# Lakonik/MVEdit

Hardware: AMD Instinct MI355X
Metric: multi-view denoise-steps/sec (32 views, 512^2) (higher is better)
Workload: dtype f16; 1 GPU; 32-view 512x512 get_noise_pred: 64 SD-1.5 UNet forwards (64x64 latents, ctx 77x768) + CFG per step; ControlNet residuals zero; views=32, latent=64, cfg=True, parallelism=views/1

## Files before the change

### include/mvedit_amd.h

```cpp
#ifndef MVEDIT_AMD_H
#define MVEDIT_AMD_H

#include <stdint.h>
#include <stddef.h>

#ifdef __cplusplus
extern "C" {
#endif

#define MVE_API __attribute__((visibility("default")))

typedef enum {
    MVE_OK = 0,
    MVE_ERR_ARG = -1,
    MVE_ERR_HIP = -2,
    MVE_ERR_STATE = -3,
    MVE_ERR_NOMEM = -4
} mve_status;

typedef enum {
    MVE_F32 = 0,
    MVE_F16 = 1,
    MVE_BF16 = 2,
    MVE_I32 = 3,
// ... 5 lines not shown
MVE_API int mve_device_info(int* n_cu, int* wave_size, char* arch, int arch_len);


MVE_API int mve_near_far_from_aabb(const float* d_rays_o, const float* d_rays_d, const float* d_aabb,
                                   uint32_t N, float min_near, float* d_nears, float* d_fars, void* stream);

MVE_API int mve_morton3d(const int32_t* d_coords, uint32_t N, int32_t* d_indices, void* stream);
MVE_API int mve_morton3d_invert(const int32_t* d_indices, uint32_t N, int32_t* d_coords, void* stream);

MVE_API int mve_packbits(const float* d_grid, uint32_t n_bytes, float density_thresh, uint8_t* d_bitfield, void* stream);

MVE_API int mve_flatten_rays(const int32_t* d_rays, uint32_t N, uint32_t M, int32_t* d_res, void* stream);

MVE_API size_t mve_march_scratch_bytes(uint32_t N);
MVE_API int mve_march_rays_train_count(const float* d_rays_o, const float* d_rays_d, const uint8_t* d_grid,
                                       float bound, int contract, float dt_gamma, uint32_t max_steps,
                                       uint32_t N, uint32_t C, uint32_t H,
                                       const float* d_nears, const float* d_fars, const float* d_noises,
                                       int32_t* d_rays, int32_t* d_total, void* d_scratch, void* stream);
MVE_API int mve_march_rays_train_write(const float* d_rays_o, const float* d_rays_d, const uint8_t* d_grid,
                                       float bound, int contract, float dt_gamma, uint32_t max_steps,
                                       uint32_t N, uint32_t C, uint32_t H,
                                       const float* d_nears, const float* d_fars, const float* d_noises,
                                       const int32_t* d_rays, uint32_t capacity,
                                       float* d_xyzs, float* d_dirs, float* d_ts, void* stream);

MVE_API int mve_march_rays_train_clamp(const int32_t* d_rays, uint32_t N, const int32_t* d_total, uint32_t capacity,
                                       int32_t* d_n_samples, int32_t* d_count, int32_t* d_overflow, void* stream);

MVE_API int mve_composite_rays_train_forward(const float* d_sigmas, const float* d_rgbs, const float* d_ts,
                                             const int32_t* d_rays, uint32_t M, uint32_t N, float T_thresh, int binarize,
                                             float* d_weights, float* d_weights_sum, float* d_depth, float* d_image,
                                             void* stream);
MVE_API int mve_composite_rays_train_backward(const float* d_grad_weights, const float* d_grad_weights_sum,
                                              const float* d_grad_depth, const float* d_grad_image,
                                              const float* d_sigmas, const float* d_rgbs, const float* d_ts,
                                              const int32_t* d_rays, const float* d_weights_sum, const float* d_depth,
                                              const float* d_image, uint32_t M, uint32_t N, float T_thresh, int binarize,
                                              float* d_grad_sigmas, float* d_grad_rgbs, void* stream);

MVE_API int mve_march_rays(uint32_t n_alive, uint32_t n_step, const int32_t* d_rays_alive, const float* d_rays_t,
                           const float* d_rays_o, const float* d_rays_d, float bound, int contract, float dt_gamma,
                           uint32_t max_steps, uint32_t C, uint32_t H, const uint8_t* d_grid,
                           const float* d_nears, const float* d_fars,
                           float* d_xyzs, float* d_dirs, float* d_ts, const float* d_noises, void* stream);
MVE_API int mve_composite_rays(uint32_t n_alive, uint32_t n_step, float T_thresh, int binarize,
                               int32_t* d_rays_alive, float* d_rays_t, const float* d_sigmas, const float* d_rgbs,
                               const float* d_ts, float* d_weights_sum, float* d_depth, float* d_image, void* stream);

MVE_API int mve_compact_alive(const int32_t* d_rays_alive, uint32_t n_alive, int32_t* d_out, int32_t* d_n_out,
                              void* d_scratch, void* stream);

MVE_API size_t mve_cull_scratch_bytes(uint32_t M);
MVE_API int mve_cull_samples(const float* d_weights, uint32_t M, float threshold, const int32_t* d_rays, uint32_t N,
                             const float* d_xyzs, const float* d_dirs, const float* d_ts, float* d_out_xyzs, float* d_out_dirs,
                             float* d_out_ts, int32_t* d_out_rays, int32_t* d_pref, int32_t* d_n_out, void* d_scratch,
                             void* stream);
MVE_API int mve_cull_samples_n(const float* d_weights, uint32_t capacity, const int32_t* d_count, float threshold, const int32_t* d_rays,
                               uint32_t N, const float* d_xyzs, const float* d_dirs, const float* d_ts, float* d_out_xyzs,
                               float* d_out_dirs, float* d_out_ts, int32_t* d_out_rays, int32_t* d_pref, int32_t* d_n_out,
                               void* d_scratch, void* stream);

MVE_API int mve_density_grid_points(const int32_t* d_coords, const float* d_noise, uint32_t N, uint32_t grid_size, float bound,
                                    float* d_xyzs, int32_t* d_indices, void* stream);
MVE_API size_t mve_density_grid_scratch_bytes(uint32_t n_cells);
MVE_API int mve_density_grid_update(float* d_density_grid, float* d_tmp_grid, uint32_t n_cells, const float* d_sigmas,
                                    const int32_t* d_indices, uint32_t N, float decay, float* d_mean_density, void* d_scratch,
                                    void* stream);


#define MVE_GEMM_GEGLU   1
#define MVE_GEMM_OUT_F32 2
#define MVE_CONV_W_CHUNK64 4
#define MVE_GEMM_NO_SPLITK 8
#define MVE_CONV_PAD_BR 32
#define MVE_GEMM_RES_AFTER_SCALE 16

MVE_API int mve_gemm(int dtype, const void* d_A, int lda, const void* d_W, int ldw, void* d_out, int ldc,
                     int M, int N, int K, const float* d_bias, const float* d_rowvec, int ldrv, int rows_per_vec,
                     const void* d_residual, int ldr, int flags, float out_scale, void* d_workspace,
                     size_t workspace_bytes, int rows_per_image, void* stream);

MVE_API int mve_gemm_tune(int big_min_blocks);
MVE_API int mve_gemm_red_tune(int on);
MVE_API int mve_gemm_deep_tune(int max_blocks);
MVE_API int mve_gemm_effective_splitk(int M, int N, int K, int rows_per_image);
#define MVE_PLAN_RESIDUAL 1
#define MVE_PLAN_RESIDUAL_LO 2
#define MVE_PLAN_OUT_LO 4
#define MVE_PLAN_ROWVEC 8
#define MVE_PLAN_LN 16
#define MVE_PLAN_BIAS 32
#define MVE_PLAN_WORKSPACE 64
#define MVE_PLAN_SCALED 128
#define MVE_PLAN_DESCRIBE_INTS 12
MVE_API int mve_gemm_plan_describe(int kind, int M, int N, int K, int rows_per_image, int flags, int features, const int* conv_geom, int* out);

MVE_API int mve_gemm_pp_profile(void* d_buf);

MVE_API size_t mve_gemm_workspace_bytes(int M, int N, int K, int rows_per_image);

MVE_API int mve_conv3x3(int dtype, const void* d_x1, int C1, const void* d_x2, int C2, int B, int Hs, int Ws,
                        int stride, int upsample, const void* d_W, int Cout, void* d_out, int ldc,
                        const float* d_bias, const float* d_rowvec, int ldrv, const void* d_residual, int ldr,
                        int flags, float out_scale, void* d_workspace, size_t workspace_bytes, void* stream);

MVE_API int mve_conv3x3_shortcut(int dtype, const void* x1, int C1, const void* x3, int C3, const void* x4, int C4, int B, int Hs,
                                 int Ws, const void* W, int Cout, void* out, int ldc, const float* bias, const float* bias2,
                                 const void* residual, int ldr, int flags, float out_scale, void* d_workspace,
                                 size_t workspace_bytes, void* stream);

MVE_API int mve_upsample_conv_phases_supported(int C, int Cout, int B, int Hs, int Ws);
MVE_API int mve_upsample_conv_phases_tune(int one_launch);
MVE_API size_t mve_upsample_conv_phases_workspace_bytes(int C, int Cout, int B, int Hs, int Ws);
MVE_API int mve_pack_upsample_phase_weights(int src_dtype, int dst_dtype, const void* d_w_oihw, int Cout, int C, void* d_W4, void* stream);
MVE_API int mve_upsample_conv_phases(int dtype, const void* d_x, int C, int B, int Hs, int Ws, const void* d_W4, int Cout, void* d_out,
                                     const float* d_bias, int flags, void* d_workspace, size_t workspace_bytes, void* d_out_lo, void* stream);

MVE_API int mve_gemm_pair(int dtype, const void* d_A, int lda, const void* d_W, int ldw, void* d_out, int ldc,
                          int M, int N, int K, const float* d_bias, const float* d_rowvec, int ldrv, int rows_per_vec,
                          const void* d_residual, int ldr, int flags, float out_scale, void* d_workspace,
                          size_t workspace_bytes, int rows_per_image, const void* d_residual_lo, void* d_out_lo, void* stream);

MVE_API int mve_gemm_pair_ln(int dtype, const void* d_A, int lda, const void* d_W, int ldw, void* d_out, int ldc, int M, int N, int K,
                             const float* d_bias, const void* d_residual, int ldr, void* d_workspace, size_t workspace_bytes, int rows_per_image,
                             const void* d_residual_lo, void* d_out_lo, void* d_ln_out, int ld_ln, const float* d_ln_gamma, const float* d_ln_beta,
                             float ln_eps, void* stream);
MVE_API int mve_gemm_ln_fuse_tune(int on);

MVE_API int mve_conv3x3_pair(int dtype, const void* x1, int C1, const void* x2, int C2, int B, int Hs, int Ws, int stride,
                             int upsample, const void* W, int Cout, void* out, int ldc, const float* bias, const float* rowvec,
                             int ldrv, const void* residual, int ldr, int flags, float out_scale, void* d_workspace,
                             size_t workspace_bytes, const void* d_residual_lo, void* d_out_lo, void* stream);
MVE_API int mve_conv3x3_shortcut_pair(int dtype, const void* x1, int C1, const void* x3, int C3, const void* x4, int C4, int B, int Hs,
                                      int Ws, const void* W, int Cout, void* out, int ldc, const float* bias, const float* bias2,
                                      int flags, float out_scale, void* d_workspace, size_t workspace_bytes, void* d_out_lo, void* stream);
MVE_API int mve_groupnorm_silu_pair(int dtype, const void* d_x1, int C1, const void* d_x2, int C2, int B, int HW, int G,
                                    float eps, const float* d_gamma, const float* d_beta, int silu, void* d_out,
                                    void* d_workspace, const void* d_x1_lo, const void* d_x2_lo, void* stream);
MVE_API int mve_layernorm_pair(int dtype, const void* d_x, int ldx, void* d_y, int ldy, int M, int C,
                               const float* d_gamma, const float* d_beta, float eps, const void* d_x_lo, void* stream);
MVE_API int mve_axpy_pair(int dtype, const void* d_a, const void* d_a_lo, const void* d_b, float alpha, void* d_y, void* d_y_lo, size_t n, void* stream);

MVE_API int mve_mxfp8_packed_k(int K);
MVE_API int mve_mxfp8_quantize(int dtype, const void* d_x, int ldx, int R, int K, uint8_t* d_q, uint8_t* d_e, void* stream);
MVE_API int mve_mxfp8_gemm(const uint8_t* d_aq, const uint8_t* d_ae, const uint8_t* d_wq, const uint8_t* d_we, int M, int N, int K, int out_dtype,
                           void* d_out, int ldc, const float* d_bias, const void* d_residual, int ldr, void* stream);

MVE_API int mve_attention(int dtype, const void* d_Q, int ldq, const void* d_K, int ldk, const void* d_V, int ldv,
                          const void* d_K2, int ldk2, const void* d_V2, int ldv2, void* d_O, int ldo,
                          int B, int Lq, int Lk, int Lk2, int heads, int head_dim, float scale, void* stream);
MVE_API int mve_attention_tune(int variant);
MVE_API int mve_attention_profile(unsigned long long* out4);
MVE_API int mve_attention_prescaled(int dtype, const void* d_Q, int ldq, const void* d_K, int ldk, const void* d_V, int ldv,
                                    const void* d_K2, int ldk2, const void* d_V2, int ldv2, void* d_O, int ldo,
                                    int B, int Lq, int Lk, int Lk2, int heads, int head_dim, void* stream);


MVE_API int mve_attention_causal(int dtype, const void* d_Q, int ldq, const void* d_K, int ldk, const void* d_V, int ldv, void* d_O, int ldo,
                                 int B, int L, int heads, int head_dim, float scale, void* stream);
MVE_API int mve_clip_embed(int dtype, const int32_t* d_ids, const void* d_tok, const void* d_pos, void* d_out, int B, int L, int C, int vocab,
                           int max_pos, void* stream);
#define MVE_ACT_QUICK_GELU 0
#define MVE_ACT_GELU 1
MVE_API int mve_act(int dtype, int kind, const void* d_x, void* d_y, size_t n, void* stream);
MVE_API int mve_clip_pool(int dtype, const void* d_x, const int32_t* d_ids, void* d_out, int B, int L, int C, int eos_token_id, void* stream);


MVE_API int mve_clip_patchify(int dtype, const void* d_pixels, int B, int H, int W, int P, void* d_rows, int ld, void* stream);
MVE_API int mve_clip_vision_embed(int dtype, const void* d_patch, const void* d_cls, const void* d_pos, void* d_out, int B, int G2, int C, void* stream);


MVE_API int mve_dpt_stem_rows(int dtype, const void* d_pixels, int B, int S, void* d_rows, int ld, void* stream);
MVE_API int mve_dpt_maxpool(int dtype, const void* d_x, int B, int H, int W, int C, void* d_y, void* stream);
MVE_API int mve_dpt_gather_s2(int dtype, const void* d_x, int B, int H, int W, int C, void* d_y, void* stream);
MVE_API int mve_dpt_upsample2x(int dtype, const void* d_x, int B, int H, int W, int C, void* d_y, void* stream);
MVE_API int mve_dpt_add_relu(int dtype, const void* d_a, const void* d_b, void* d_y, size_t n, void* stream);


MVE_API int mve_loftr_stem_rows(int dtype, const void* d_pixels, int B, int H, int W, void* d_rows, int ld, void* stream);
MVE_API int mve_loftr_leaky_relu(int dtype, const void* d_x, void* d_y, size_t n, float slope, void* stream);
MVE_API int mve_loftr_pos_add(int dtype, const void* d_x, const float* d_pos, void* d_y, int B, int HW, int C, void* stream);

MVE_API size_t mve_linattn_workspace_bytes(int B, int S, int H, int D);
MVE_API int mve_linattn_kv(int dtype, const void* d_k, int ldk, const void* d_v, int ldv, int B, int S, int H, int D, float* d_kv, void* d_workspace,
                           size_t workspace_bytes, void* stream);
MVE_API int mve_linattn_apply(int dtype, const void* d_q, int ldq, const float* d_kv, void* d_out, int ldo, int B, int L, int H, int D, float eps,
                              void* stream);

MVE_API int mve_dsmax_stats(const float* d_sim, int N, int L, int S, int ld, float* d_row_stats, float* d_col_stats, void* stream);
MVE_API int mve_dsmax_conf(const float* d_sim, int N, int L, int S, int ld, const float* d_row_stats, const float* d_col_stats, float* d_conf, void* stream);
MVE_API size_t mve_dsmax_select_workspace_bytes(int N, int L, int S);
MVE_API int mve_dsmax_select(const float* d_conf, int N, int H0, int W0, int H1, int W1, float thr, int border, float scale, int64_t* d_b_ids,
                             int64_t* d_i_ids, int64_t* d_j_ids, float* d_mconf, float* d_mkpts0_c, float* d_mkpts1_c, int* d_count, void* d_workspace,
                             size_t workspace_bytes, void* stream);

MVE_API int mve_loftr_unfold(int dtype, const void* d_feat, int N, int Hf, int Wf, int C, const int64_t* d_b_ids, const int64_t* d_ids, int M, void* d_rows,
                             void* stream);
MVE_API int mve_loftr_ln_add(int dtype, const void* d_o, int ldo, const void* d_x, int ldx, void* d_y, int ldy, int M, int C, const float* d_gamma,
                             const float* d_beta, float eps, void* stream);
MVE_API int mve_loftr_gather_rows(int dtype, const void* d_feat, int N, int L, int C, const int64_t* d_b_ids, const int64_t* d_ids, int M, void* d_rows,
                                  void* stream);
MVE_API int mve_loftr_fine_match(int dtype, const void* d_feat0, const void* d_feat1, int M, int C, const float* d_mkpts1_c, float radius, float* d_expec_f,
                                 float* d_mkpts1_f, void* stream);


MVE_API int mve_attention_relpos(int dtype, const void* d_Q, int ldq, const void* d_K, int ldk, const void* d_V, int ldv, const void* d_rel_h,
                                 const void* d_rel_w, void* d_O, int ldo, int NS, int gh, int gw, int heads, int head_dim, float scale, void* stream);
MVE_API int mve_sam_window_partition(int dtype, const void* d_x, int B, int G, int C, int window, void* d_win, void* stream);
MVE_API int mve_sam_window_unpartition(int dtype, const void* d_win, int B, int G, int C, int window, void* d_x, void* stream);
MVE_API int mve_sam_pos_add(int dtype, const void* d_x, const void* d_pos, void* d_y, int B, int HW, int C, void* stream);


MVE_API int mve_sam_preprocess(int dtype, const uint8_t* d_image, int h, int w, int S, const float* pixel_mean, const float* pixel_std, void* d_out, void* stream);
MVE_API int mve_sam_dense_pe(const float* d_gaussian, float* d_out, int G, int C, void* stream);
MVE_API int mve_sam_prompt_tokens(const float* d_boxes, const float* d_points, const int32_t* d_labels, int N, int n_points, const float* d_gaussian,
                                  const float* d_point_embed, const float* d_not_a_point, const float* d_iou_token, const float* d_mask_tokens, int num_mask_tokens,
                                  int C, float image_size, float* d_out, int T, void* stream);
MVE_API int mve_sam_src(int dtype, const void* d_embedding, const float* d_no_mask_embed, float* d_out, int N, int P, int C, int G, void* stream);
MVE_API int mve_gemm_f32(const float* d_A, int lda, const float* d_W, int ldw, const float* d_bias, const float* d_res, int ldr, float* d_out, int ldc, int M, int N,
                         int K, int relu, void* stream);
MVE_API int mve_attention_f32(const float* d_Q, int ldq, const float* d_K, int ldk, const float* d_V, int ldv, float* d_O, int ldo, int NB, int Lq, int Lk,
                              int heads, int head_dim, float scale, void* stream);
MVE_API int mve_layernorm_f32(const float* d_x, float* d_y, int rows, int C, const float* d_gamma, const float* d_beta, float eps, void* stream);
MVE_API int mve_add_rows_f32(const float* d_x, const float* d_pe, float* d_y, int rows, int C, int period_rows, void* stream);
MVE_API int mve_sam_upscale(const float* d_x, const float* d_W4, const float* d_bias, const float* d_ln_gamma, const float* d_ln_beta, float eps, float* d_tmp,
                            float* d_out, int N, int Gi, int Cin, int Cout, int mode, void* stream);
MVE_API int mve_sam_token_mlps(const float* d_queries, int N, int T, int C, int hidden, int out_dim, int num_mask_tokens, const float* d_w0, const float* d_b0,
                               const float* d_w1, const float* d_b1, const float* d_w2, const float* d_b2, float* d_hyper, float* d_iou, void* stream);
MVE_API int mve_sam_mask_product(const float* d_hyper, const float* d_up, float* d_low_res, int N, int num_mask_tokens, int Cu, int pixels, void* stream);
MVE_API int mve_sam_postprocess(const float* d_low_res, int planes, int L, int S, int h_in, int w_in, int H, int W, float mask_threshold, uint8_t* d_masks,
                                float* d_logits, void* stream);

MVE_API int mve_groupnorm_tune(int fused_max_hw);
MVE_API size_t mve_groupnorm_workspace_bytes(int B, int HW, int C, int G);
MVE_API int mve_groupnorm_silu(int dtype, const void* d_x1, int C1, const void* d_x2, int C2, int B, int HW, int G,
                               float eps, const float* d_gamma, const float* d_beta, int silu, void* d_out,
                               void* d_workspace, void* stream);

MVE_API int mve_layernorm(int dtype, const void* d_x, int ldx, void* d_y, int ldy, int M, int C,
                          const float* d_gamma, const float* d_beta, float eps, void* stream);

MVE_API int mve_nchw_to_nhwc(int dst_dtype, int src_dtype, const void* d_x, int B, int C, int H, int W, int Cpad,
                             void* d_y, void* stream);
MVE_API int mve_nhwc_to_nchw(int dst_dtype, int src_dtype, const void* d_x, int ld, int B, int C, int H, int W,
                             void* d_y, void* stream);
MVE_API int mve_timestep_embedding(int dtype, const float* d_t, int B, int dim, void* d_out, void* stream);
MVE_API int mve_text_time_embedding(int dtype, const void* d_text_embeds, int text_dtype, int text_dim, const float* d_time_ids, int n_ids,
                                    int time_embed_dim, int B, void* d_out, void* stream);
MVE_API int mve_silu(int dtype, const void* d_x, void* d_y, size_t n, void* stream);
MVE_API int mve_axpy(int dtype, const void* d_a, const void* d_b, float alpha, void* d_y, size_t n, void* stream);
MVE_API int mve_softmax_rows(int dtype, const float* d_scores, size_t lds, int M, int N, void* d_probs, size_t ldp, void* stream);
MVE_API int mve_cfg_combine(const float* d_uncond, const float* d_text, float guidance_scale, float* d_out, size_t n,
                            void* stream);
MVE_API int mve_x0_prediction(const float* d_latents_scaled, const float* d_noise_pred, float sqrt_alpha_bar,
                              float sqrt_one_minus_alpha_bar, size_t n, float* d_x0, void* stream);

MVE_API int mve_tonemap_lut(const float* d_x, size_t n, const float* d_lut_x, const float* d_lut_y, int steps, int inverse, int linear,
                            float* d_out, void* stream);
MVE_API int mve_tonemap_lut_backward(const float* d_x, const float* d_grad_out, size_t n, const float* d_lut_x, const float* d_lut_y,
                                     int steps, int inverse, int linear, float* d_grad_x, void* stream);

MVE_API int mve_gaussian_blur(const float* d_x, int planes, int H, int W, int ksize, float sigma, int adjoint, const float* d_base,
                              float offset, float* d_tmp, float* d_out, void* stream);

MVE_API int mve_sh_encode(const float* d_inputs, uint32_t B, int degree, float* d_outputs, float* d_dy_dx, void* stream);
MVE_API int mve_sh_encode_backward(const float* d_grad, const float* d_dy_dx, uint32_t B, int degree, float* d_grad_inputs, void* stream);
MVE_API int mve_shade_views(const float* d_rgba, const float* d_normal_fg, const float* d_cam_lights, uint32_t n_views,
                            uint32_t pix_per_view, float ambient_light, float bg_color, const float* d_lut_x, const float* d_lut_y,
                            int steps, float* d_image, void* stream);
MVE_API int mve_shade_points(const float* d_albedo, const float* d_normal, const float* d_lights, size_t N, float ambient_light,
                             const float* d_lut_x, const float* d_lut_y, int steps, float* d_out, const float* d_grad_out,
                             float* d_grad_albedo, float* d_grad_normal, void* stream);

typedef struct MveReconLossDesc {
    int32_t P, ps, shaded, is_init, lut_steps;
    float ambient_light, bg_color, normal_bg[3];
    float pixel_loss_weight, normal_reg_weight, depth_weight, entropy_weight, bg_width;
    const float *d_lut_x, *d_lut_y;
    const float *d_image, *d_weights_sum, *d_depth;
    const float *d_weights, *d_ts;
    uint32_t M;
    const float *d_target_dir, *d_target_rgbs, *d_target_m, *d_target_n, *d_target_depth;
    const float *d_patch_w, *d_patch_lights;
} MveReconLossDesc;
MVE_API size_t mve_recon_loss_workspace_bytes(int P, int ps, uint32_t M);
MVE_API int mve_recon_loss_forward(const MveReconLossDesc* desc, void* d_ws, size_t ws_bytes, float* d_losses, float* d_out_rgbs,
                                   float* d_out_normals, void* stream);
MVE_API int mve_recon_loss_backward(const MveReconLossDesc* desc, void* d_ws, size_t ws_bytes, const float* d_g_out_rgbs,
                                    const float* d_g_out_normals, const float* d_g_loss, float* d_g_image, float* d_g_weights_sum, float* d_g_depth,
                                    float* d_g_weights, void* stream);
MVE_API int mve_recon_loss_forward_n(const MveReconLossDesc* desc, const int32_t* d_count, void* d_ws, size_t ws_bytes, float* d_losses,
                                     float* d_out_rgbs, float* d_out_normals, void* stream);
MVE_API int mve_recon_loss_backward_n(const MveReconLossDesc* desc, const int32_t* d_count, void* d_ws, size_t ws_bytes,
                                      const float* d_g_out_rgbs, const float* d_g_out_normals, const float* d_g_loss, float* d_g_image,
                                      float* d_g_weights_sum, float* d_g_depth, float* d_g_weights, void* stream);

typedef struct MveMeshLossDesc {
    int32_t n, size, mesh_is_simplified;
    float normal_bg[3];
    float pixel_loss_weight, normal_reg_weight;
    const float *d_rgba, *d_normal, *d_depth;
    const float *d_target_dir, *d_target_rgbs, *d_target_m_erode, *d_target_m_blur, *d_target_n;
    const float *d_view_w;
} MveMeshLossDesc;
MVE_API size_t mve_mesh_loss_workspace_bytes(int n, int size);
// ... 344 lines not shown
```

### mvedit_amd/_lib.py

```python
import ctypes
import os
import re

import torch

_HERE = os.path.dirname(os.path.abspath(__file__))
HEADER = os.path.join(os.path.dirname(_HERE), 'include', 'mvedit_amd.h')
LIB_PATH = os.path.join(_HERE, 'libmvedit_amd.so' if not os.environ.get('MVE_LIB_TAG') else f"libmvedit_amd_{os.environ['MVE_LIB_TAG']}.so")

_CTYPE = {
    'void': None,
    'int': ctypes.c_int,
    'float': ctypes.c_float,
    'double': ctypes.c_double,
    'size_t': ctypes.c_size_t,
    'uint32_t': ctypes.c_uint32,
    'int32_t': ctypes.c_int32,
    'uint64_t': ctypes.c_uint64,
    'int64_t': ctypes.c_int64,
    'uint8_t': ctypes.c_uint8,
    'char': ctypes.c_char,
}


class MveError(RuntimeError):
    pass


def parse_header(path=HEADER):
    src = open(path).read()
    src = re.sub(r'/\*.*?\*/', ' ', src, flags=re.S)
    src = re.sub(r'//[^\n]*', ' ', src)
    protos = {}
    for m in re.finditer(r'MVE_API\s+([\w\s\*]+?)\s*\b(mve_\w+)\s*\(([^;{]*?)\)\s*;', src, flags=re.S):
        ret, name, args = m.group(1).strip(), m.group(2), m.group(3).strip()
        arglist = []
        if args and args != 'void':
            for a in args.split(','):
                a = ' '.join(a.split())
                mm = re.match(r'(.*?)(\w+)$', a)
                arglist.append((mm.group(1).strip(), mm.group(2)))
        protos[name] = (ret, arglist)
    return protos


def _to_ctype(tstr):
    t = tstr.replace('const', ' ').strip()
    stars = t.count('*')
    base = t.replace('*', ' ').split()
    base = base[-1] if base else 'void'
    if stars:
        if base == 'char' and stars == 1:
            return ctypes.c_char_p
        return ctypes.c_void_p
    if base in _CTYPE:
        return _CTYPE[base]
    return ctypes.c_int


PROTOS = parse_header()

if not os.path.exists(LIB_PATH):
    raise ImportError(
        f'{LIB_PATH} is missing: build it with `python -m mvedit_amd.build` '
        '(mvedit_amd has no CPU or PyTorch fallback for its HIP kernels)')

_dll = ctypes.CDLL(LIB_PATH, mode=ctypes.RTLD_LOCAL)

for _name, (_ret, _args) in PROTOS.items():
    try:
        _fn = getattr(_dll, _name)
    except AttributeError as e:
        raise ImportError(f'libmvedit_amd.so does not export {_name} declared in mvedit_amd.h') from e
    _fn.restype = _to_ctype(_ret)
    _fn.argtypes = [_to_ctype(t) for t, _ in _args]

_dll.mve_last_error.restype = ctypes.c_char_p


def last_error():
    return _dll.mve_last_error().decode()


def call(name, *args):
    rc = getattr(_dll, name)(*args)
    if rc < 0:
        raise MveError(f'{name} failed ({rc}): {last_error()}')
    return rc


def raw(name):
    return getattr(_dll, name)


def ptr(t):
    if t is None:
        return None
    return ctypes.c_void_p(t.data_ptr())


def stream_ptr(device=None):
    return ctypes.c_void_p(torch.cuda.current_stream(device).cuda_stream)
```

### mvedit_amd/csrc/attention.hip

```cpp
#include "common.h"

#include <stdlib.h>
#include <type_traits>

namespace {

constexpr int NT = 256;

struct AttnParams {
    const void* Q; const void* K; const void* V; const void* K2; const void* V2; void* O;
    int ldq, ldk, ldv, ldk2, ldv2, ldo;
    int B, Lq, Lk, Lk2, heads;
    float scale_log2e;
    int prescaled;
    const int* skip_if;
};

template <int DP, bool KSW2> __device__ __forceinline__ int k_perm(int row, int pc) {
    if constexpr (DP == 64) return pc ^ ((row >> 1) & 7);
    else if constexpr (KSW2) return pc ^ (((row >> 3) & 1) << 1);
    else return pc ^ ((row >> 2) & 3);
}
template <int DP, bool KSW2> __device__ __forceinline__ int k_swz(int row, int chunk) {
    return row * (DP * 2) + (k_perm<DP, KSW2>(row, chunk) << 4);
// ... 554 lines not shown
            for (int r2 = 0; r2 < 8; ++r2) {
                float e0, e1;
                if constexpr (PRE && (ABL & 8) != 0) {
                    e0 = sk[2 * r2]; e1 = sk[2 * r2 + 1];
                } else if constexpr (PRE) {
                    e0 = __builtin_amdgcn_exp2f(sk[2 * r2]);
                    e1 = __builtin_amdgcn_exp2f(sk[2 * r2 + 1]);
                } else {
                    e0 = __builtin_amdgcn_exp2f(__builtin_fmaf(sk[2 * r2], sc, nm));
                    e1 = __builtin_amdgcn_exp2f(__builtin_fmaf(sk[2 * r2 + 1], sc, nm));
                }
                pk[r2] = __builtin_bit_cast(unsigned, __builtin_convertvector(f32x2{e0, e1}, T2));
            }
#pragma unroll
            for (int v = 0; v < 4; ++v) {
                const int ai = v < 2 ? v : v + 2;
                if constexpr ((ABL & 512) != 0) { pb.w[kb][0][v] = pk[ai]; pb.w[kb][1][v] = pk[ai + 2]; continue; }
                const auto r = __builtin_amdgcn_permlane16_swap(pk[ai], pk[ai + 2], false, false);
                pb.w[kb][0][v] = r[0];
                pb.w[kb][1][v] = r[1];
            }
        }
        return pb;
    };

    auto pv = [&](const unsigned char* St, const PB& pb) {
#pragma unroll
        for (int kb = 0; kb < 2; ++kb) {
            s16x4 lo[3], up[3];
            const unsigned va0 = (unsigned)(uintptr_t)(lds_ptr_t)(St + v_off + kb * 32 * V_ROW);
            if constexpr ((ABL & 256) != 0) {
#pragma unroll
                for (int i = 0; i < 3; ++i) { lo[i] = __builtin_bit_cast(s16x4, u32x2{pb.w[kb][0][i], va0}); up[i] = __builtin_bit_cast(s16x4, u32x2{va0, pb.w[kb][1][i]}); }
            } else {
                typedef __attribute__((address_space(3))) s16x4* lp;
#pragma unroll
                for (int i = 0; i < 3; ++i) {
                    lo[i] = __builtin_amdgcn_ds_read_tr16_b64_v4i16((lp)(lds_ptr_t)(St + v_off + kb * 32 * V_ROW + 32 * i));
                    up[i] = __builtin_amdgcn_ds_read_tr16_b64_v4i16((lp)(lds_ptr_t)(St + v_off + kb * 32 * V_ROW + 32 * i + 16 * V_ROW));
                }
            }
#pragma unroll
            for (int i = 0; i < 3; ++i) {
                const V8 va = __builtin_bit_cast(V8, __builtin_shufflevector(lo[i], up[i], 0, 1, 2, 3, 4, 5, 6, 7));
#pragma unroll
                for (int f = 0; f < 2; ++f) {
                    const u32x4 pw = {pb.w[kb][f][0], pb.w[kb][f][1], pb.w[kb][f][2], pb.w[kb][f][3]};
                    if constexpr ((ABL & 64) != 0) { asm volatile("" : "+v"(oacc[i][f]) : "v"(va), "v"(pw)); continue; }
                    oacc[i][f] = Tag::mfma16(va, __builtin_bit_cast(V8, pw), oacc[i][f]);
                }
            }
        }
    };

    auto wait_sync = [&](int keep) {
        if constexpr ((ABL & 3) == 3) { asm volatile("s_waitcnt lgkmcnt(0)" ::: "memory"); return; }
        else if constexpr ((ABL & 1) != 0) { asm volatile("s_waitcnt vmcnt(0)\n\ts_waitcnt lgkmcnt(0)" ::: "memory"); return; }
        else if constexpr ((ABL & 2) != 0) { asm volatile("s_waitcnt lgkmcnt(0)\n\ts_barrier" ::: "memory"); return; }
        if (keep >= 3) asm volatile("s_waitcnt vmcnt(3)\n\ts_waitcnt lgkmcnt(0)\n\ts_barrier" ::: "memory");
        else if (keep == 2) asm volatile("s_waitcnt vmcnt(2)\n\ts_waitcnt lgkmcnt(0)\n\ts_barrier" ::: "memory");
        else if (keep == 1) asm volatile("s_waitcnt vmcnt(1)\n\ts_waitcnt lgkmcnt(0)\n\ts_barrier" ::: "memory");
        else asm volatile("s_waitcnt vmcnt(0)\n\ts_waitcnt lgkmcnt(0)\n\ts_barrier" ::: "memory");
    };
    auto next_stage = [&](int off) { return off + STAGE == NST * STAGE ? 0 : off + STAGE; };

    if constexpr (!PIPE) {
        constexpr int PD = NST - 1;
        static_assert(DMA_PER_WAVE * (PD - 1) <= 3, "wait_sync covers at most three outstanding instructions");
#pragma unroll
        for (int i = 0; i < PD; ++i)
            if (i < n_tiles) dma(i, i * STAGE);
        asm volatile("" : "+v"(qf[0]), "+v"(qf[1]), "+v"(qf[2]));
        wait_sync(n_mine * ((n_tiles < PD ? n_tiles : PD) - 1));
        int cur = 0, nxt = PD * STAGE;
        for (int t = 0; t < n_full; ++t) {
            if (t + PD < n_tiles) dma(t + PD, nxt);
            S2 s = qk(smem + cur);
            softmax_max(s, t * KB, std::false_type{}, t == 0);
            const PB pb = softmax_exp(s);
            pv(smem + cur, pb);
            const int last_issued = t + PD < n_tiles ? t + PD : n_tiles - 1;
            wait_sync(last_issued > t + 1 ? n_mine * (last_issued - (t + 1)) : 0);
            nxt = cur;
            cur = next_stage(cur);
        }
        if (n_full < n_tiles) {
            S2 s = qk(smem + cur);
            softmax_max(s, n_full * KB, std::true_type{}, n_full == 0);
            const PB pb = softmax_exp(s);
            pv(smem + cur, pb);
        }
    } else {
        static_assert(NST >= 3, "the pipelined loop needs the next tile's K resident");
        constexpr int PD = NST - 1;
        static_assert(DMA_PER_WAVE * (PD - 2) <= 3, "wait_sync covers at most three outstanding instructions");
#pragma unroll
        for (int i = 0; i < PD; ++i)
            if (i < n_tiles) dma(i, i * STAGE);
        asm volatile("" : "+v"(qf[0]), "+v"(qf[1]), "+v"(qf[2]));
        {
            const int issued = n_tiles < PD ? n_tiles : PD;
            wait_sync(issued > 2 ? n_mine * (issued - 2) : 0);
        }
        int cur = 0, nx1 = STAGE, nxt = (PD % NST) * STAGE;
        S2 sA = qk(smem), sB;
        const int n_main = n_tiles - 1;
        auto step = [&](S2& sc_, S2& sn_, int t) {
            if (t + PD < n_tiles) dma(t + PD, nxt);
            softmax_max(sc_, t * KB, std::false_type{}, t == 0);
            sn_ = qk(smem + nx1);
            const PB pb = softmax_exp(sc_);
            pv(smem + cur, pb);
            const int last_issued = t + PD < n_tiles ? t + PD : n_tiles - 1;
            wait_sync(last_issued > t + 2 ? n_mine * (last_issued - (t + 2)) : 0);
            nxt = cur; cur = nx1; nx1 = next_stage(nx1);
        };
        int t = 0;
        for (; t + 2 <= n_main; t += 2) { step(sA, sB, t); step(sB, sA, t + 1); }
        if (t < n_main) { step(sA, sB, t); sA = sB; ++t; }
        if (n_full < n_tiles) softmax_max(sA, t * KB, std::true_type{}, t == 0);
        else softmax_max(sA, t * KB, std::false_type{}, t == 0);
        const PB pb = softmax_exp(sA);
        pv(smem + cur, pb);
    }

#pragma unroll
    for (int f = 0; f < 2; ++f) {
        const float l = __shfl(oacc[2][f][0], 32 + l16, 64);
        const float inv = 1.0f / l;
        const int q = q_base + f * 16 + l16;
        if (q < p.Lq) {
            T* orow = reinterpret_cast<T*>(p.O) + ((size_t)b * p.Lq + q) * p.ldo + h * D;
#pragma unroll
            for (int i = 0; i < 3; ++i) {
                const int dv = i * 16 + g * 4;
                if (dv < D) {
                    T4 o4;
#pragma unroll
                    for (int r = 0; r < 4; ++r) o4[r] = Tag::from_f32(oacc[i][f][r] * inv);
                    *reinterpret_cast<T4*>(orow + dv) = o4;
                }
            }
        }
    }
    if constexpr ((ABL & 1024) != 0) {
        unsigned long long t1, r1;
        asm volatile("s_memtime %0\n\ts_memrealtime %1\n\ts_waitcnt lgkmcnt(0)" : "=s"(t1), "=s"(r1) :: "memory");
        if (lane == 0 && (blockIdx.x & 63) == 5) {
            atomicAdd(&g_attn_prof[0], t1 - prof_t0);
            atomicAdd(&g_attn_prof[1], r1 - prof_r0);
            atomicAdd(&g_attn_prof[2], 1ull);
        }
    }
}

int g_attn_variant = 9;
int g_attn_ablate = 0;

template <class Tag, int D>
int launch(const AttnParams& p, hipStream_t s) {
    if constexpr (D == 40) {
        if (g_attn_variant >= 8 && g_attn_variant <= 15) {
            const int var = g_attn_variant;
            const bool w8 = var == 9 || var == 11 || var >= 14;
            const unsigned grid3 = (unsigned)(((p.Lq + (w8 ? 255 : 127)) / (w8 ? 256 : 128)) * p.heads * p.B);
#define MVE_A3P(SEG, NW_, NST_, WPS_, PRE_, PIPE_) k_attention3<Tag, SEG, NW_, NST_, WPS_, PRE_, PIPE_><<<grid3, 64 * NW_, 0, s>>>(p)
#define MVE_A3(NW_, NST_, WPS_, PIPE_) do { \
                if (p.Lk2 > 0) { if (p.prescaled && !PIPE_) MVE_A3P(true, NW_, NST_, WPS_, (!PIPE_), PIPE_); else MVE_A3P(true, NW_, NST_, WPS_, false, PIPE_); } \
                else { if (p.prescaled && !PIPE_) MVE_A3P(false, NW_, NST_, WPS_, (!PIPE_), PIPE_); else MVE_A3P(false, NW_, NST_, WPS_, false, PIPE_); } } while (0)
#ifdef MVE_ATTN_LAB
            if (g_attn_ablate != 0) {
                if constexpr (std::is_same<Tag, F16Tag>::value) {
                    if (p.Lk2 == 0 && p.prescaled) {
                        const unsigned grid9 = (unsigned)(((p.Lq + 255) / 256) * p.heads * p.B);
                        bool hit = true;
                        switch (g_attn_ablate) {
#define MVE_ABL(A) case A: k_attention3<Tag, false, 8, 2, 4, true, false, (A) | 1024><<<grid9, 512, 0, s>>>(p); break;
                            MVE_ABL(2048) MVE_ABL(1) MVE_ABL(3) MVE_ABL(7) MVE_ABL(8) MVE_ABL(16) MVE_ABL(24) MVE_ABL(32) MVE_ABL(64) MVE_ABL(96) MVE_ABL(128) MVE_ABL(256)
                            MVE_ABL(384) MVE_ABL(512) MVE_ABL(536) MVE_ABL(927) MVE_ABL(480) MVE_ABL(1023)
#undef MVE_ABL
                            default: hit = false;
                        }
                        if (hit) { MVE_LAUNCH_CHECK(); return MVE_OK; }
                    }
                }
            }
#endif
            switch (var) {
                case 8: MVE_A3(4, 2, 4, false); break;
                case 9: MVE_A3(8, 2, 4, false); break;
                case 10: MVE_A3(4, 3, 4, false); break;
                case 11: MVE_A3(8, 3, 4, false); break;
                case 12: MVE_A3(4, 3, 3, true); break;
                case 13: MVE_A3(4, 4, 3, true); break;
                case 14: MVE_A3(8, 3, 2, true); break;
                default: MVE_A3(8, 4, 2, true); break;
            }
#undef MVE_A3P
#undef MVE_A3
            MVE_LAUNCH_CHECK();
            return MVE_OK;
        }
        if (g_attn_variant == 1 && p.Lk2 == 0) {
            const unsigned grid1 = (unsigned)(((p.Lq + 63) / 64) * p.heads * p.B);
            k_attention2<Tag, D, false, 1, 64, 3><<<grid1, NT, 0, s>>>(p);
            MVE_LAUNCH_CHECK();
            return MVE_OK;
        }
    }
    constexpr int QB = 128;
    const unsigned grid = (unsigned)(((p.Lq + QB - 1) / QB) * p.heads * p.B);
    const int var = g_attn_variant >= 8 ? ((D == 80 || D == 160) ? 6 : 4) : g_attn_variant;
    if constexpr (D == 80 || D == 160) {
        if ((var == 2 || var == 6) && p.Lk2 == 0) {
            if (var == 6) k_attention2<Tag, D, false, 2, 0, 0, true, true><<<grid, NT, 0, s>>>(p);
            else k_attention2<Tag, D, false, 2, 0, 0, true><<<grid, NT, 0, s>>>(p);
            MVE_LAUNCH_CHECK();
            return MVE_OK;
        }
    }
    if ((var == 4 || var == 6) && p.Lk2 == 0) {
        k_attention2<Tag, D, false, 2, 0, 0, false, true><<<grid, NT, 0, s>>>(p);
        MVE_LAUNCH_CHECK();
        return MVE_OK;
    }
    if (p.Lk2 > 0) k_attention2<Tag, D, true><<<grid, NT, 0, s>>>(p);
    else k_attention2<Tag, D, false><<<grid, NT, 0, s>>>(p);
    MVE_LAUNCH_CHECK();
    return MVE_OK;
}

template <class Tag>
int dispatch_d(const AttnParams& p, int d, hipStream_t s) {
    switch (d) {
        case 40: return launch<Tag, 40>(p, s);
        case 64: return launch<Tag, 64>(p, s);
        case 80: return launch<Tag, 80>(p, s);
        case 160: return launch<Tag, 160>(p, s);
        default:
            mve_set_error("attention: unsupported head dim %d (supported: 40, 64, 80, 160)", d);
            return MVE_ERR_ARG;
    }
}

}

extern "C" int mve_attention_profile(unsigned long long* out4) {
    MVE_CHECK(out4, MVE_ERR_ARG, "attention_profile: null pointer");
#ifndef MVE_ATTN_LAB
    mve_set_error("attention_profile: the timing-only ablation kernels are compiled into development builds only (MVE_ATTN_LAB=1 python -m mvedit_amd.build)");
    return MVE_ERR_STATE;
#endif
    MVE_HIP(hipDeviceSynchronize());
    MVE_HIP(hipMemcpyFromSymbol(out4, HIP_SYMBOL(g_attn_prof), 4 * sizeof(unsigned long long)));
    const unsigned long long z[4] = {0ull, 0ull, 0ull, 0ull};
    MVE_HIP(hipMemcpyToSymbol(HIP_SYMBOL(g_attn_prof), z, sizeof(z)));
    return MVE_OK;
}

extern "C" int mve_attention_tune(int variant) {
    const int old = g_attn_variant | (g_attn_ablate << 8);
#ifndef MVE_ATTN_LAB
    if (variant >= 256) { mve_set_error("attention_tune: ablation bits (8-19) need a development build (MVE_ATTN_LAB=1)"); return MVE_ERR_ARG; }
#endif
    if (variant >= 0) { g_attn_variant = variant & 255; g_attn_ablate = (variant >> 8) & 4095; }
    return old;
}

static int attention_entry(int dtype, const void* Q, int ldq, const void* K, int ldk, const void* V, int ldv,
                           const void* K2, int ldk2, const void* V2, int ldv2, void* O, int ldo, int B, int Lq,
                           int Lk, int Lk2, int heads, int head_dim, float scale, int prescaled, void* stream) {
    if (B == 0 || Lq == 0) return MVE_OK;
    MVE_CHECK(Q && K && V && O, MVE_ERR_ARG, "attention: null pointer");
    MVE_CHECK(Lk > 0 && Lk2 >= 0 && heads > 0, MVE_ERR_ARG, "attention: bad sizes Lk=%d Lk2=%d heads=%d", Lk, Lk2, heads);
    MVE_CHECK(Lk2 == 0 || (K2 && V2), MVE_ERR_ARG, "attention: second KV segment has null pointers");
    MVE_CHECK(ldq % 8 == 0 && ldk % 8 == 0 && ldv % 8 == 0 && ldo % 4 == 0 && (Lk2 == 0 || (ldk2 % 8 == 0 && ldv2 % 8 == 0)),
              MVE_ERR_ARG, "attention: leading dimensions must be multiples of 8");
    AttnParams p;
    p.Q = Q; p.K = K; p.V = V; p.K2 = K2; p.V2 = V2; p.O = O;
    p.ldq = ldq; p.ldk = ldk; p.ldv = ldv; p.ldk2 = ldk2; p.ldv2 = ldv2; p.ldo = ldo;
    p.B = B; p.Lq = Lq; p.Lk = Lk; p.Lk2 = Lk2; p.heads = heads;
    p.scale_log2e = prescaled ? 1.0f : scale * 1.4426950408889634f;
    p.prescaled = prescaled;
    p.skip_if = mve_skip_second_half();
    MVE_CHECK(!p.skip_if || B % 2 == 0, MVE_ERR_ARG, "attention: the second-half predicate needs an even batch (B=%d)", B);
    if (dtype == MVE_F16) return dispatch_d<F16Tag>(p, head_dim, (hipStream_t)stream);
    if (dtype == MVE_BF16) return dispatch_d<BF16Tag>(p, head_dim, (hipStream_t)stream);
    mve_set_error("attention: unsupported dtype %d", dtype);
    return MVE_ERR_ARG;
}

extern "C" int mve_attention(int dtype, const void* Q, int ldq, const void* K, int ldk, const void* V, int ldv,
                             const void* K2, int ldk2, const void* V2, int ldv2, void* O, int ldo, int B, int Lq,
                             int Lk, int Lk2, int heads, int head_dim, float scale, void* stream) {
    return attention_entry(dtype, Q, ldq, K, ldk, V, ldv, K2, ldk2, V2, ldv2, O, ldo, B, Lq, Lk, Lk2, heads, head_dim, scale, 0, stream);
}

extern "C" int mve_attention_prescaled(int dtype, const void* Q, int ldq, const void* K, int ldk, const void* V, int ldv,
                                       const void* K2, int ldk2, const void* V2, int ldv2, void* O, int ldo, int B, int Lq,
                                       int Lk, int Lk2, int heads, int head_dim, void* stream) {
    return attention_entry(dtype, Q, ldq, K, ldk, V, ldv, K2, ldk2, V2, ldv2, O, ldo, B, Lq, Lk, Lk2, heads, head_dim, 1.0f, 1, stream);
}
```

Measured before the change: 15.94 denoise-steps/s.

## Add single-pass short-KV attention kernel for cross-attention with Lk<=96

Adds a dedicated attention kernel for short key sequences (Lk<=96, e.g. 77-token text context). The whole K/V for a group of heads is loaded into LDS once, and each wave processes query tiles with a single-pass softmax and no online rescaling. It uses transposed LDS reads for V and a ones-column trick to get the row sum. This targets the loop and rescale overhead of the general flash kernel on cross-attention, and it is enabled by default with an environment switch to turn it off. It adds code complexity and depends on heuristic chunking of the grid.

```diff
diff --git a/include/mvedit_amd.h b/include/mvedit_amd.h
--- a/include/mvedit_amd.h
+++ b/include/mvedit_amd.h
@@ -181,6 +181,8 @@
                           int B, int Lq, int Lk, int Lk2, int heads, int head_dim, float scale, void* stream);
 MVE_API int mve_attention_tune(int variant);
 MVE_API int mve_attention_profile(unsigned long long* out4);
+MVE_API int mve_attention_short(int on);
+MVE_API int mve_attention_last_path(void);
 MVE_API int mve_attention_prescaled(int dtype, const void* d_Q, int ldq, const void* d_K, int ldk, const void* d_V, int ldv,
                                     const void* d_K2, int ldk2, const void* d_V2, int ldv2, void* d_O, int ldo,
                                     int B, int Lq, int Lk, int Lk2, int heads, int head_dim, void* stream);
diff --git a/mvedit_amd/_lib.py b/mvedit_amd/_lib.py
--- a/mvedit_amd/_lib.py
+++ b/mvedit_amd/_lib.py
@@ -93,6 +93,14 @@
     return getattr(_dll, name)
 
 
+def attention_short(on=-1):
+    return _dll.mve_attention_short(int(on))
+
+
+def attention_last_path():
+    return _dll.mve_attention_last_path()
+
+
 def ptr(t):
     if t is None:
         return None
diff --git a/mvedit_amd/csrc/attention.hip b/mvedit_amd/csrc/attention.hip
--- a/mvedit_amd/csrc/attention.hip
+++ b/mvedit_amd/csrc/attention.hip
@@ -730,6 +730,273 @@
             atomicAdd(&g_attn_prof[2], 1ull);
         }
     }
+}
+
+template <int D> struct ShortCfg {
+    static constexpr int QF = D > 80 ? 1 : 2;
+    static constexpr int QT = 16 * QF;
+    static constexpr int PD = D > 80 ? 1 : 2;
+    static constexpr int HG = 160 / D, WPH = 4 / HG;
+    static constexpr int KR = 96;
+    static constexpr int DP = (D + 31) / 32 * 32, KS = DP / 32, DC = D / 8, DVF = (D + 15) / 16;
+    static constexpr bool ONES = (D % 16) != 0;
+    static constexpr int K_ROW = D * 2 + (D == 40 ? 0 : 16);
+    static constexpr int V_ROW = D == 40 ? 96 : (D == 80 ? 160 : 352);
+    static constexpr int VC = ONES ? DC + 1 : DC;
+    static constexpr int HEAD_BYTES = KR * (K_ROW + V_ROW);
+    static constexpr int LDS_BYTES = HG * HEAD_BYTES;
+};
+
+template <class Tag, int D, bool ST16, int NKF>
+__global__ __launch_bounds__(NT, 2) void k_attention_short(const AttnParams p, const int chunk_tiles, const int n_chunks) {
+    typedef ShortCfg<D> C;
+    constexpr int QF = C::QF, QT = C::QT, HG = C::HG, WPH = C::WPH, KR = C::KR, KS = C::KS, DC = C::DC, DVF = C::DVF;
+    constexpr int NKK = (NKF + 1) / 2;
+    static_assert(NKF >= 1 && NKF * 16 <= KR, "key fragments");
+    constexpr int K_ROW = C::K_ROW, V_ROW = C::V_ROW, VC = C::VC, HEAD_BYTES = C::HEAD_BYTES;
+    constexpr bool ONES = C::ONES;
+    typedef typename Tag::V8 V8;
+    typedef typename Tag::T T;
+    typedef T T4 __attribute__((ext_vector_type(4)));
+
+    extern __shared__ __attribute__((aligned(16))) unsigned char smem_short[];
+
+    const int tid = threadIdx.x, lane = tid & 63;
+    const int wv = __builtin_amdgcn_readfirstlane(tid >> 6);
+    const int g = lane >> 4, l16 = lane & 15;
+
+    const int nhg = (p.heads + HG - 1) / HG;
+    const unsigned bid = mve_xcd_remap(blockIdx.x, gridDim.x);
+    const int hg = bid % nhg;
+    const int ch = (bid / nhg) % n_chunks;
+    const int b = bid / (nhg * n_chunks);
+    const int h0 = hg * HG;
+    if (mve_second_half_skipped(p.skip_if, 2 * b >= p.B)) return;
+
+    const int hh = wv / WPH, sub = wv % WPH;
+    const int h = h0 + hh;
+    const int q_tiles = (p.Lq + QT - 1) / QT;
+    const int t_end = h >= p.heads ? 0 : ((ch + 1) * chunk_tiles < q_tiles ? (ch + 1) * chunk_tiles : q_tiles);
+    int t = ch * chunk_tiles + sub;
+
+    const unsigned char* Kh = smem_short + hh * HEAD_BYTES;
+    const unsigned char* Vh = Kh + KR * K_ROW;
+    int koff[KS];
+#pragma unroll
+    for (int ks = 0; ks < KS; ++ks) { const int c = ks * 4 + g; koff[ks] = l16 * K_ROW + (c < DC ? c : 0) * 16; }
+    const int voff = (lane >> 2) * V_ROW + (lane & 3) * 8;
+    const float sc = p.scale_log2e;
+    const int kl = p.Lk - g * 4;
+
+    const T* Qb = reinterpret_cast<const T*>(p.Q) + (size_t)b * p.Lq * p.ldq + (h < p.heads ? h : 0) * D;
+    T* Ob = reinterpret_cast<T*>(p.O) + (size_t)b * p.Lq * p.ldo + (h < p.heads ? h : 0) * D;
+
+    auto load_q = [&](int tile, V8 (&q)[QF][KS]) {
+        tile = tile < t_end ? tile : t_end - 1;
+        tile = tile > 0 ? tile : 0;
+#pragma unroll
+        for (int f = 0; f < QF; ++f) {
+            int qi = tile * QT + f * 16 + l16;
+            qi = qi < p.Lq ? qi : p.Lq - 1;
+            const T* row = Qb + (size_t)qi * p.ldq;
+#pragma unroll
+            for (int ks = 0; ks < KS; ++ks) {
+                const int c = ks * 4 + g;
+                q[f][ks] = __builtin_bit_cast(V8, *reinterpret_cast<const u32x4*>(row + (c < DC ? c : 0) * 8));
+            }
+        }
+    };
+
+    const unsigned qmask = (KS - 1) * 4 + g < DC ? ~0u : 0u;
+    auto tile_body = [&](const V8 (&qin)[QF][KS], int tile) {
+        V8 qf[QF][KS];
+#pragma unroll
+        for (int f = 0; f < QF; ++f)
+#pragma unroll
+            for (int ks = 0; ks < KS; ++ks) {
+                if (DC % 4 != 0 && ks == KS - 1) {
+                    u32x4 v = __builtin_bit_cast(u32x4, qin[f][ks]);
+#pragma unroll
+                    for (int e = 0; e < 4; ++e) v[e] &= qmask;
+                    qf[f][ks] = __builtin_bit_cast(V8, v);
+                } else qf[f][ks] = qin[f][ks];
+            }
+        f32x4 s[NKF][QF];
+#pragma unroll
+        for (int kf = 0; kf < NKF; ++kf)
+#pragma unroll
+            for (int f = 0; f < QF; ++f) s[kf][f] = f32x4{0.f, 0.f, 0.f, 0.f};
+#pragma unroll
+        for (int ks = 0; ks < KS; ++ks)
+#pragma unroll
+            for (int kf = 0; kf < NKF; ++kf) {
+                const V8 ka = *reinterpret_cast<const V8*>(Kh + koff[ks] + kf * 16 * K_ROW);
+#pragma unroll
+                for (int f = 0; f < QF; ++f) s[kf][f] = Tag::mfma16(ka, qf[f][ks], s[kf][f]);
+            }
+#pragma unroll
+        for (int kf = 0; kf < NKF; ++kf)
+            if (kf * 16 + 16 > p.Lk) {
+#pragma unroll
+                for (int r = 0; r < 4; ++r)
+                    if (kf * 16 + r >= kl) {
+#pragma unroll
+                        for (int f = 0; f < QF; ++f) s[kf][f][r] = -INFINITY;
+                    }
+            }
+        V8 pf[QF][NKK];
+        float lsum[QF];
+#pragma unroll
+        for (int f = 0; f < QF; ++f) {
+            float mx = s[0][f][0];
+#pragma unroll
+            for (int kf = 0; kf < NKF; ++kf)
+#pragma unroll
+                for (int r = 0; r < 4; ++r) mx = fmaxf(mx, s[kf][f][r]);
+            mx = mve_max_xor32(mve_max_xor16(mx));
+            const float nm = -mx * sc;
+            float psum = 0.f;
+#pragma unroll
+            for (int kk = 0; kk < NKK; ++kk) {
+                f32x8 e;
+#pragma unroll
+                for (int r = 0; r < 4; ++r) {
+                    e[r] = __builtin_amdgcn_exp2f(__builtin_fmaf(s[2 * kk][f][r], sc, nm));
+                    e[4 + r] = 2 * kk + 1 < NKF ? __builtin_amdgcn_exp2f(__builtin_fmaf(s[2 * kk + 1 < NKF ? 2 * kk + 1 : 0][f][r], sc, nm)) : 0.f;
+                }
+                if constexpr (!ONES) {
+#pragma unroll
+                    for (int r = 0; r < 8; ++r) psum += e[r];
+                }
+                pf[f][kk] = __builtin_convertvector(e, V8);
+            }
+            lsum[f] = psum;
+        }
+        f32x4 oacc[DVF][QF];
+#pragma unroll
+        for (int i = 0; i < DVF; ++i)
+#pragma unroll
+            for (int f = 0; f < QF; ++f) oacc[i][f] = f32x4{0.f, 0.f, 0.f, 0.f};
+        typedef __attribute__((address_space(3))) s16x4* lp;
+#pragma unroll
+        for (int kk = 0; kk < NKK; ++kk)
+#pragma unroll
+            for (int i = 0; i < DVF; ++i) {
+                const s16x4 lo = __builtin_amdgcn_ds_read_tr16_b64_v4i16((lp)(lds_ptr_t)(Vh + voff + kk * 32 * V_ROW + 32 * i));
+                const s16x4 up = __builtin_amdgcn_ds_read_tr16_b64_v4i16((lp)(lds_ptr_t)(Vh + voff + (kk * 32 + 16) * V_ROW + 32 * i));
+                const V8 va = __builtin_bit_cast(V8, __builtin_shufflevector(lo, up, 0, 1, 2, 3, 4, 5, 6, 7));
+#pragma unroll
+                for (int f = 0; f < QF; ++f) oacc[i][f] = Tag::mfma16(va, pf[f][kk], oacc[i][f]);
+            }
+        float inv[QF];
+#pragma unroll
+        for (int f = 0; f < QF; ++f) {
+            float l;
+            if constexpr (ONES) {
+                l = __shfl(oacc[DVF - 1][f][(D % 16) % 4], ((D % 16) / 4) * 16 + l16, 64);
+            } else {
+                l = lsum[f];
+                l += __shfl_xor(l, 16, 64);
+                l += __shfl_xor(l, 32, 64);
+            }
+            inv[f] = 1.0f / l;
+        }
+        const int q0 = tile * QT + l16;
+        if constexpr (!ST16) {
+#pragma unroll
+            for (int f = 0; f < QF; ++f) {
+                const int q = q0 + f * 16 < p.Lq ? q0 + f * 16 : p.Lq - 1;
+                T* orow = Ob + (size_t)q * p.ldo;
+#pragma unroll
+                for (int i = 0; i < DVF; ++i) {
+                    const int dv = i * 16 + g * 4;
+                    T4 o4;
+#pragma unroll
+                    for (int r = 0; r < 4; ++r) o4[r] = Tag::from_f32(oacc[i][f][r] * inv[f]);
+                    if (dv < D) *reinterpret_cast<T4*>(orow + dv) = o4;
+                }
+            }
+        } else {
+            auto pack = [&](int i, int f) -> u32x2 {
+                T4 o4;
+#pragma unroll
+                for (int r = 0; r < 4; ++r) o4[r] = Tag::from_f32(oacc[i][f][r] * inv[f]);
+                return __builtin_bit_cast(u32x2, o4);
+            };
+            auto swap16 = [&](u32x2 a, u32x2 bb) -> u32x4 {
+                const auto r0 = __builtin_amdgcn_permlane16_swap(a[0], bb[0], false, false);
+                const auto r1 = __builtin_amdgcn_permlane16_swap(a[1], bb[1], false, false);
+                return u32x4{r0[0], r1[0], r0[1], r1[1]};
+            };
+            if constexpr (QF == 2) {
+                const int q = q0 + (g & 1) * 16 < p.Lq ? q0 + (g & 1) * 16 : p.Lq - 1;
+                T* orow = Ob + (size_t)q * p.ldo + (g >> 1) * 8;
+#pragma unroll
+                for (int i = 0; i < DVF; ++i) {
+                    const u32x4 o8 = swap16(pack(i, 0), pack(i, 1));
+                    if (i * 16 + 16 <= D || (g >> 1) == 0) *reinterpret_cast<u32x4*>(orow + i * 16) = o8;
+                }
+            } else {
+                static_assert(QF == 2 || DVF % 2 == 0, "the 16-byte store pairs dv fragments");
+                const int q = q0 < p.Lq ? q0 : p.Lq - 1;
+                T* orow = Ob + (size_t)q * p.ldo + (g & 1) * 16 + (g >> 1) * 8;
+#pragma unroll
+                for (int j = 0; j < DVF / 2; ++j) *reinterpret_cast<u32x4*>(orow + j * 32) = swap16(pack(2 * j, 0), pack(2 * j + 1, 0));
+            }
+        }
+    };
+
+    constexpr int PD = C::PD;
+    V8 qa[QF][KS], qb[QF][KS], qc[QF][KS];
+
+    {
+        constexpr int KCH = KR * DC, VCH = KR * VC, PER_HEAD = KCH + VCH, TOTAL = HG * PER_HEAD, UNR = (TOTAL + NT - 1) / NT;
+        const T* Kg = reinterpret_cast<const T*>(p.K) + (size_t)b * p.Lk * p.ldk + h0 * D;
+        const T* Vg = reinterpret_cast<const T*>(p.V) + (size_t)b * p.Lk * p.ldv + h0 * D;
+        u32x4 ones_chunk = {0u, 0u, 0u, 0u};
+        if constexpr (ONES) ones_chunk[0] = __builtin_bit_cast(unsigned short, Tag::from_f32(1.0f));
+        u32x4 w[UNR];
+        int dst[UNR];
+#pragma unroll
+        for (int u = 0; u < UNR; ++u) {
+            int idx = u * NT + tid;
+            const bool in = idx < TOTAL;
+            idx = in ? idx : TOTAL - 1;
+            const int fh = idx / PER_HEAD, rem = idx - fh * PER_HEAD;
+            const bool isk = rem < KCH;
+            const int rv = isk ? rem : rem - KCH;
+            const int r = isk ? rv / DC : rv / VC;
+            const int c = rv - r * (isk ? DC : VC);
+            const bool pad = c >= DC;
+            const bool live = h0 + fh < p.heads && r < p.Lk && !pad;
+            const int rs = r < p.Lk ? r : p.Lk - 1, hs = h0 + fh < p.heads ? fh : 0, cs = pad ? DC - 1 : c;
+            const T* src = (isk ? Kg + (size_t)rs * p.ldk : Vg + (size_t)rs * p.ldv) + hs * D + cs * 8;
+            w[u] = *reinterpret_cast<const u32x4*>(src);
+            const int o = fh * HEAD_BYTES + (isk ? r * K_ROW : KR * K_ROW + r * V_ROW) + c * 16;
+            dst[u] = in ? (o | (live ? 1 << 30 : 0) | (pad ? 1 << 29 : 0)) : -1;
+        }
+        load_q(t, qa);
+        if constexpr (PD == 2) load_q(t + WPH, qb);
+#pragma unroll
+        for (int u = 0; u < UNR; ++u) {
+            u32x4 v;
+#pragma unroll
+            for (int e = 0; e < 4; ++e) v[e] = (dst[u] & (1 << 30)) ? w[u][e] : ((dst[u] & (1 << 29)) ? ones_chunk[e] : 0u);
+            if (dst[u] >= 0) *reinterpret_cast<u32x4*>(smem_short + (dst[u] & 0xffffff)) = v;
+        }
+    }
+    __syncthreads();
+    if (t >= t_end) return;
+
+#define MVE_SHORT_STEP(CUR, NXT) load_q(t + PD * WPH, NXT); tile_body(CUR, t); if ((t += WPH) >= t_end) return
+    if constexpr (PD == 2) {
+        MVE_SHORT_STEP(qa, qc); MVE_SHORT_STEP(qb, qa); MVE_SHORT_STEP(qc, qb);
+        for (;;) { MVE_SHORT_STEP(qa, qc); MVE_SHORT_STEP(qb, qa); MVE_SHORT_STEP(qc, qb); }
+    } else {
+        MVE_SHORT_STEP(qa, qb); MVE_SHORT_STEP(qb, qa);
+        for (;;) { MVE_SHORT_STEP(qa, qb); MVE_SHORT_STEP(qb, qa); }
+    }
+#undef MVE_SHORT_STEP
 }
 
 int g_attn_variant = 9;
@@ -808,8 +1075,53 @@
     return MVE_OK;
 }
 
+int g_attn_short = -1;
+int g_attn_last_short = 0;
+
+int attn_short_switch() {
+    if (g_attn_short < 0) {
+        const char* e = getenv("MVE_ATTN_SHORT");
+        g_attn_short = (e && atoi(e) == 0) ? 0 : 1;
+    }
+    return g_attn_short;
+}
+
+bool attn_short_applies(const AttnParams& p, int d) {
+    return p.Lk2 == 0 && p.Lk <= 96 && (d == 40 || d == 80 || d == 160) && attn_short_switch() != 0;
+}
+
+template <class Tag, int D>
+int launch_short(const AttnParams& p, hipStream_t s) {
+    typedef ShortCfg<D> C;
+    const int q_tiles = (p.Lq + C::QT - 1) / C::QT;
+    const int nhg = (p.heads + C::HG - 1) / C::HG;
+    const long long per = (long long)p.B * nhg;
+    int n_chunks = per >= 512 ? 1 : (int)(512 / per);
+    const int max_chunks = (q_tiles + C::WPH - 1) / C::WPH;
+    if (n_chunks > max_chunks) n_chunks = max_chunks;
+    int chunk_tiles = (q_tiles + n_chunks - 1) / n_chunks;
+    chunk_tiles = (chunk_tiles + C::WPH - 1) / C::WPH * C::WPH;
+    n_chunks = (q_tiles + chunk_tiles - 1) / chunk_tiles;
+    const long long nblk = per * n_chunks;
+    MVE_CHECK(nblk < (1ll << 31), MVE_ERR_ARG, "attention: grid too large (B=%d heads=%d)", p.B, p.heads);
+    const bool st16 = p.ldo % 8 == 0 && (reinterpret_cast<uintptr_t>(p.O) & 15) == 0;
+    const dim3 grid((unsigned)nblk), block(NT);
+    if (p.Lk <= 80) {
+        if (st16) return mve_launch_dyn_lds<k_attention_short<Tag, D, true, 5>>(grid, block, C::LDS_BYTES, s, p, chunk_tiles, n_chunks);
+        return mve_launch_dyn_lds<k_attention_short<Tag, D, false, 5>>(grid, block, C::LDS_BYTES, s, p, chunk_tiles, n_chunks);
+    }
+    if (st16) return mve_launch_dyn_lds<k_attention_short<Tag, D, true, 6>>(grid, block, C::LDS_BYTES, s, p, chunk_tiles, n_chunks);
+    return mve_launch_dyn_lds<k_attention_short<Tag, D, false, 6>>(grid, block, C::LDS_BYTES, s, p, chunk_tiles, n_chunks);
+}
+
 template <class Tag>
 int dispatch_d(const AttnParams& p, int d, hipStream_t s) {
+    g_attn_last_short = attn_short_applies(p, d) ? 1 : 0;
+    if (g_attn_last_short) {
+        if (d == 40) return launch_short<Tag, 40>(p, s);
+        if (d == 80) return launch_short<Tag, 80>(p, s);
+        return launch_short<Tag, 160>(p, s);
+    }
     switch (d) {
         case 40: return launch<Tag, 40>(p, s);
         case 64: return launch<Tag, 64>(p, s);
@@ -844,6 +1156,14 @@
     if (variant >= 0) { g_attn_variant = variant & 255; g_attn_ablate = (variant >> 8) & 4095; }
     return old;
 }
+
+extern "C" int mve_attention_short(int on) {
+    const int old = attn_short_switch();
+    if (on >= 0) g_attn_short = on ? 1 : 0;
+    return old;
+}
+
+extern "C" int mve_attention_last_path(void) { return g_attn_last_short; }
 
 static int attention_entry(int dtype, const void* Q, int ldq, const void* K, int ldk, const void* V, int ldv,
                            const void* K2, int ldk2, const void* V2, int ldv2, void* O, int ldo, int B, int Lq,
```

Result: no change. 16.06 denoise-steps/s (median of 6 runs) (+0.8%).
